# jameschapman19/cca_zoo

Measured on AMD Instinct MI355X. Metric: CCA fit()/sec at n=1e6 d=4096 k=64, higher is better.
Workload: dtype f32

## Files before the change

cca_zoo_amd/csrc/gram.hip:

```cpp
#include <algorithm>
#include <cstdio>
#include <cstdlib>
#include <cstring>
#include <thread>
#include <vector>

#include "hip_common.h"
#include "gram_map.h"

namespace ccz {

typedef float v16f32 __attribute__((ext_vector_type(16)));
typedef float v4f32 __attribute__((ext_vector_type(4)));
typedef double v4f64 __attribute__((ext_vector_type(4)));
typedef double v2f64 __attribute__((ext_vector_type(2)));

constexpr int BK = 16;

typedef const float __attribute__((address_space(1)))* gptr_f32;
typedef const double __attribute__((address_space(1)))* gptr_f64;

typedef unsigned int v4u32 __attribute__((ext_vector_type(4)));

constexpr int T32 = 256;
// ... 687 lines not shown
                                                      double* __restrict__ zero_me, int64_t nzero) {
  __shared__ int last;
  if (zero_me && blockIdx.y == 0)
    for (int64_t e = int64_t(blockIdx.x) * 256 + threadIdx.x; e < nzero; e += int64_t(gridDim.x) * 256) zero_me[e] = 0.0;
  const int64_t j = int64_t(blockIdx.x) * 256 + threadIdx.x;
  const int64_t r0 = int64_t(blockIdx.y) * rows_per_block;
  const int64_t r1 = min(n, r0 + rows_per_block);
  if (j < D) {
    int a = 0;
    while (a + 1 < cv.m && j >= cv.off[a + 1]) ++a;
    const float* X = cv.data[a] + (j - cv.off[a]);
    const int64_t ld = cv.ld[a];
    double a0 = 0.0, a1 = 0.0, a2 = 0.0, a3 = 0.0;
    int64_t r = r0;
    for (; r + 3 < r1; r += 4) {
      a0 += double(X[(r + 0) * ld]); a1 += double(X[(r + 1) * ld]);
      a2 += double(X[(r + 2) * ld]); a3 += double(X[(r + 3) * ld]);
    }
    for (; r < r1; ++r) a0 += double(X[r * ld]);
    st_shared(part + int64_t(blockIdx.y) * D + j, (a0 + a1) + (a2 + a3));
  }
  asm volatile("s_waitcnt vmcnt(0)" ::: "memory");
  __syncthreads();
  if (threadIdx.x == 0)
    last = __hip_atomic_fetch_add(counters + blockIdx.x, 1u, __ATOMIC_RELAXED, __HIP_MEMORY_SCOPE_AGENT) == gridDim.y - 1 ? 1 : 0;
  __syncthreads();
  if (!last) return;
  if (threadIdx.x == 0) __hip_atomic_store(counters + blockIdx.x, 0u, __ATOMIC_RELAXED, __HIP_MEMORY_SCOPE_AGENT);
  if (j >= D) return;
  double t0 = 0.0, t1 = 0.0, t2 = 0.0, t3 = 0.0;
  int rb = 0;
  const int nrb = int(gridDim.y);
  for (; rb + 3 < nrb; rb += 4) {
    t0 += ld_shared(part + int64_t(rb) * D + j); t1 += ld_shared(part + int64_t(rb + 1) * D + j);
    t2 += ld_shared(part + int64_t(rb + 2) * D + j); t3 += ld_shared(part + int64_t(rb + 3) * D + j);
  }
  for (; rb < nrb; ++rb) t0 += ld_shared(part + int64_t(rb) * D + j);
  const double sj = (t0 + t1) + (t2 + t3);
  sums[j] = sj;
  pilot[j] = float(sj / double(n));
}

__global__ void k_pilot_from_sums(const double* __restrict__ s, int64_t D, double inv_n, float* __restrict__ pilot) {
  const int64_t j = int64_t(blockIdx.x) * blockDim.x + threadIdx.x;
  if (j < D) pilot[j] = float(s[j] * inv_n);
}

__global__ void k_pilot_fixup(double* __restrict__ G, int64_t D, const double* __restrict__ s_launch, double n,
                              const float* __restrict__ pilot) {
  const int64_t i = blockIdx.y;
  const int64_t j = i + int64_t(blockIdx.x) * blockDim.x + threadIdx.x;
  if (j >= D) return;
  const double pi = double(pilot[i]), pj = double(pilot[j]);
  G[i * D + j] += pi * s_launch[j] + pj * s_launch[i] - n * pi * pj;
}

__global__ __launch_bounds__(256) void k_gram_reduce(const float* __restrict__ partial, const GramTile* __restrict__ tiles, int ntiles,
                                                     int64_t ksplit, double* __restrict__ G, int64_t ldg) {
  const int tile = blockIdx.y;
  const GramTile t = tiles[tile];
  const int e = blockIdx.x * 256 + threadIdx.x;
  const int i = e >> 8, j = e & 255;
  if (i >= t.wa || j >= t.wb) return;
  double acc = 0.0;
  const float* p = partial + int64_t(tile) * (T32 * T32) + e;
  for (int64_t c = 0; c < ksplit; ++c) acc += double(p[c * int64_t(ntiles) * (T32 * T32)]);
  G[(t.out_row + i) * ldg + t.out_col + j] += acc;
}

__global__ void k_vec_add(double* __restrict__ dst, const double* __restrict__ src, int64_t n) {
  const int64_t j = int64_t(blockIdx.x) * blockDim.x + threadIdx.x;
  if (j < n) dst[j] += src[j];
}

namespace {

struct Panel {
  int view;
  int64_t col0, width, gcol0;
};

struct TileTable {
  GramTile* dev = nullptr;
  int ntiles = 0;
  bool fast = true;
  std::vector<unsigned char> diag;
};

template <typename T>
TileTable build_tile_table(ccz_ctx* c, const ccz_view* views, int n_views, void** tile_cache) {
  Impl* im = impl(c);
  hipStream_t st = stream(c);
  constexpr bool is32 = sizeof(T) == 4;
  const int tile = is32 ? T32 : T64;
  std::vector<Panel> panels;
  int64_t g0 = 0;
  bool fast = true;
  for (int v = 0; v < n_views; ++v) {
    for (int64_t c0 = 0; c0 < views[v].cols; c0 += tile)
      panels.push_back({v, c0, std::min<int64_t>(tile, views[v].cols - c0), g0 + c0});
    if (views[v].cols % tile != 0) fast = false;
    if ((views[v].ld * sizeof(T)) % 16 != 0) fast = false;
    if (reinterpret_cast<uintptr_t>(views[v].data) % 16 != 0) fast = false;
    g0 += views[v].cols;
  }
  std::vector<GramTile> tiles;
  const int np = int(panels.size());
// ... 121 lines not shown
template <typename T>
RowPlan plan_rows(ccz_ctx* c, const ccz_view* views, int n_views, int64_t n, int ntiles, bool fast) {
  Impl* im = impl(c);
  constexpr bool is32 = sizeof(T) == 4;
  static const int map_mode = [] { const char* e = getenv("CCZ_GRAM_MAP"); return e ? atoi(e) : 1; }();
  const int ncu = std::max(1, im->props.multiProcessorCount);
  static const int64_t rows_env = [] { const char* e = getenv("CCZ_GRAM_ROWS"); return e ? atoll(e) : 0LL; }();
  int64_t max_rows = rows_env > 0 ? rows_env : 16384;
  if (fast) {
    int64_t cap = max_rows;
    for (int v = 0; v < n_views; ++v)
      cap = std::min<int64_t>(cap, ((int64_t(1) << 31) - 1) / (views[v].ld * int64_t(sizeof(T))) - 128);
    if (cap < 256) fast = false; else max_rows = cap;
  }
  const int64_t gran = (is32 && fast) ? FB * FR : BK;
  int64_t rows_per_wg;
  {
    const int64_t kmin = std::max<int64_t>(1, (n + max_rows - 1) / max_rows);
    const int64_t kmax = std::max<int64_t>(kmin, std::min<int64_t>(n / 256, 8192));
    double best = 1e300;
    int64_t best_k = kmin;
    for (int64_t ks = kmin; ks <= kmax; ++ks) {
      const int64_t rows = ((n + ks - 1) / ks + gran - 1) / gran * gran;
      const bool big = int64_t(ntiles) * ks >= 16 * int64_t(ncu);
      int64_t rounds;
      double penalty = 1.0;
      if (big && map_mode == 1 && ks % 8 == 0) rounds = ((ks / 8) * int64_t(ntiles) + ncu / 8 - 1) / (ncu / 8);
      else if (big) { rounds = (int64_t((ntiles + 7) / 8) * ks + ncu / 8 - 1) / (ncu / 8); if (map_mode == 1) penalty = 1.03; }
      else rounds = (int64_t(ntiles) * ks + ncu - 1) / ncu;
      const double cost = penalty * double(rounds) * double(rows + 320);
      if (cost < best) { best = cost; best_k = ks; }
    }
    rows_per_wg = ((n + best_k - 1) / best_k + gran - 1) / gran * gran;
  }
  const int64_t ksplit = (n + rows_per_wg - 1) / rows_per_wg;
  const bool sliced = int64_t(ntiles) * ksplit >= 16 * int64_t(ncu);
  const bool xchunks = sliced && map_mode == 1 && ksplit % 8 == 0;
  const int per_xcd = xchunks ? -1 : (sliced ? (ntiles + 7) / 8 : 0);
  const int64_t nblocks = xchunks ? int64_t(ntiles) * ksplit : (sliced ? int64_t(8) * per_xcd * ksplit : int64_t(ntiles) * ksplit);
  if (nblocks > 0x7fffffffLL) fail(CCZ_EUNSUP, "gram: grid too large");

  RowPlan rp;
  rp.rows_per_wg = rows_per_wg;
  rp.ksplit = ksplit;
  rp.nblocks = nblocks;
  rp.per_xcd = per_xcd;
  rp.sliced = sliced;
  rp.fast = fast;
  return rp;
}

template <typename T>
bool launch_moments(ccz_ctx* c, const ccz_view* views, int n_views, int64_t n, double* G, double* s, int64_t D,
                    bool time_it, void** tile_cache = nullptr, int pilot_mode = 0) {
  Impl* im = impl(c);
  hipStream_t st = stream(c);
  constexpr bool is32 = sizeof(T) == 4;
  const int tile = is32 ? T32 : T64;
  const TileTable tt = build_tile_table<T>(c, views, n_views, tile_cache);
  GramTile* d_tiles = tt.dev;
  const int ntiles = tt.ntiles;
  const RowPlan rp = plan_rows<T>(c, views, n_views, n, ntiles, tt.fast);
  const bool fast = rp.fast;
  const int64_t rows_per_wg = rp.rows_per_wg, ksplit = rp.ksplit, nblocks = rp.nblocks;
  const int per_xcd = rp.per_xcd;
  const bool sliced = rp.sliced;
  const int ncu = std::max(1, im->props.multiProcessorCount);
  const size_t lds_bytes = size_t(2) * 2 * BK * tile * sizeof(T);
  static const int pilot_env = [] { const char* e = getenv("CCZ_GRAM_PILOT"); return e ? atoi(e) : -1; }();
  if (pilot_env == 0 || pilot_env == 1) pilot_mode = pilot_env == 1 ? 2 : 0;
  if (!is32) pilot_mode = 0;
  bool split = false;
  if (is32) {
    static const int route_env = [] {
      const char* e = getenv("CCZ_K1_ROUTE");
      if (!e) return 0;
      if (!strcmp(e, "fp32")) return int(CCZ_K1_FP32);
      if (!strcmp(e, "bf16x2")) return int(CCZ_K1_BF16X2);
      return 0;
    }();
    const int route = c->k1_route != CCZ_K1_AUTO ? c->k1_route : route_env;
    split = (route == CCZ_K1_BF16X2 || (route == CCZ_K1_AUTO && gram_split_worthwhile(n, D))) && n_views <= 16;
    if (split) pilot_mode = 2;
  }
  c->last_route = !is32 ? CCZ_K1_FP64 : (split ? CCZ_K1_BF16X2 : CCZ_K1_FP32);
  static const double pilot_thr = [] { const char* e = getenv("CCZ_GRAM_PILOT_RATIO"); return e ? atof(e) : 2.0; }();
  double* s_launch = s;
  double* sq = nullptr;
  if (pilot_mode != 0) {
    s_launch = static_cast<double*>(dev_alloc(c, size_t(D) * 8 * (pilot_mode == 1 ? 2 : 1)));
    zero(c, s_launch, size_t(D) * 8 * (pilot_mode == 1 ? 2 : 1));
    if (pilot_mode == 1) sq = s_launch + D;
  }
  if (time_it) CCZ_HIP(hipEventRecord(im->ev[2], st));
  int64_t off = 0;
  float* pilot = nullptr;
  if (split) {
    const int64_t nsamp = std::min<int64_t>(n, 2048), stride = n / nsamp;
    double* samp = static_cast<double*>(dev_alloc(c, size_t(D) * 8));
    zero(c, samp, size_t(D) * 8);
    for (int v = 0; v < n_views; ++v) {
      const int64_t colblocks = (views[v].cols + 255) / 256;
      int64_t rpb = 256;
      while (rpb > 16 && colblocks * ((nsamp + rpb - 1) / rpb) < 2 * int64_t(ncu)) rpb /= 2;
      dim3 grid((unsigned)colblocks, (unsigned)((nsamp + rpb - 1) / rpb));
      hipLaunchKernelGGL((k_colsum<T, false>), grid, dim3(256), 0, st, static_cast<const T*>(views[v].data), nsamp, views[v].cols,
                         views[v].ld * stride, samp + off, static_cast<double*>(nullptr), rpb);
      off += views[v].cols;
    }
    pilot = static_cast<float*>(dev_alloc(c, size_t(D) * 4));
    hipLaunchKernelGGL(k_pilot_from_sums, dim3((unsigned)((D + 255) / 256)), dim3(256), 0, st, samp, D, 1.0 / double(nsamp), pilot);
    dev_free(c, samp);
  }
  for (int v = 0; v < n_views && !split; ++v) {
    const int64_t colblocks = (views[v].cols + 255) / 256;
    int64_t rpb = 2048;
    while (rpb > 64 && colblocks * ((n + rpb - 1) / rpb) < 4 * int64_t(ncu)) rpb /= 2;
    dim3 grid((unsigned)colblocks, (unsigned)((n + rpb - 1) / rpb));
    if (sq)
      hipLaunchKernelGGL((k_colsum<T, true>), grid, dim3(256), 0, st, static_cast<const T*>(views[v].data), n, views[v].cols,
                         views[v].ld, s_launch + off, sq + off, rpb);
    else
      hipLaunchKernelGGL((k_colsum<T, false>), grid, dim3(256), 0, st, static_cast<const T*>(views[v].data), n, views[v].cols,
                         views[v].ld, s_launch + off, static_cast<double*>(nullptr), rpb);
    off += views[v].cols;
  }
  CCZ_LAUNCH_CHECK();
  if (time_it) CCZ_HIP(hipEventRecord(im->ev[3], st));
  bool use_pilot = pilot_mode == 2;
  if (pilot_mode == 1) {
    std::vector<double> hs(size_t(2) * D);
    d2h(c, hs.data(), s_launch, size_t(2) * D * 8);
    double worst = 0.0;
    for (int64_t j = 0; j < D; ++j) {
      const double mu = hs[j] / double(n), var = hs[D + j] / double(n) - mu * mu;
      if (!std::isfinite(mu) || !std::isfinite(var)) continue;
      const double sd = var > 0.0 ? std::sqrt(var) : 0.0;
      const double ratio = std::fabs(mu) <= pilot_thr * sd ? 0.0 : (sd > 0.0 ? std::fabs(mu) / sd : 1e300);
      if (ratio > worst) worst = ratio;
    }
    use_pilot = worst > pilot_thr;
  }
  if (use_pilot && !split) {
    pilot = static_cast<float*>(dev_alloc(c, size_t(D) * 4));
    hipLaunchKernelGGL(k_pilot_from_sums, dim3((unsigned)((D + 255) / 256)), dim3(256), 0, st, s_launch, D, 1.0 / double(n), pilot);
  }

  if (time_it) CCZ_HIP(hipEventRecord(im->ev[0], st));
  static const int impl_sel = [] { const char* e = getenv("CCZ_GRAM_IMPL"); return e ? atoi(e) : 1; }();
  static const int fifo_pilot_env = [] { const char* e = getenv("CCZ_GRAM_FIFO_PILOT"); return e ? atoi(e) : 1; }();
  const int64_t n_main = n / (FB * FR) * (FB * FR);
  const bool fifo_pilot = is32 && fast && impl_sel != 0 && use_pilot && fifo_pilot_env != 0 && sliced && n_main >= rows_per_wg;
  float* partial = nullptr;
  const bool staged32 = is32 && !(fast && impl_sel != 0 && !use_pilot) && !fifo_pilot;
  if (staged32 && ksplit >= 2 && !sliced && !split) {
    static const int64_t partial_cap = [] { const char* e = getenv("CCZ_GRAM_PARTIAL_MB"); return (e ? atoll(e) : 192LL) << 20; }();
    const int64_t bytes = ksplit * int64_t(ntiles) * T32 * T32 * 4;
    if (bytes <= partial_cap) partial = static_cast<float*>(dev_alloc(c, size_t(bytes)));
  }
  if (split) {
    gram_split_f32(c, views, n_views, n, G, D, pilot, s_launch, time_it);
  } else if (is32) {
    if (fifo_pilot) {
      const size_t fifo_bytes = size_t(4) * FR * FSLOT;
      CCZ_HIP(hipFuncSetAttribute(reinterpret_cast<const void*>(&k_gram_f32_fifo<true>), hipFuncAttributeMaxDynamicSharedMemorySize, int(fifo_bytes)));
      hipLaunchKernelGGL(k_gram_f32_fifo<true>, dim3((unsigned)nblocks), dim3(256), fifo_bytes, st, d_tiles, ntiles, per_xcd, ksplit, n_main,
                         rows_per_wg, G, D, pilot);
      if (n_main < n) {
        CCZ_HIP(hipFuncSetAttribute(reinterpret_cast<const void*>(&k_gram_f32<true>), hipFuncAttributeMaxDynamicSharedMemorySize, int(lds_bytes)));
        hipLaunchKernelGGL(k_gram_f32<true>, dim3((unsigned)ntiles), dim3(256), lds_bytes, st, d_tiles, ntiles, 0, int64_t(1), n, int64_t(FB * FR), G, D,
                           pilot, static_cast<float*>(nullptr), n_main);
      }
    } else if (fast && impl_sel != 0 && !use_pilot) {
      const size_t fifo_bytes = size_t(4) * FR * FSLOT;
      CCZ_HIP(hipFuncSetAttribute(reinterpret_cast<const void*>(&k_gram_f32_fifo<false>), hipFuncAttributeMaxDynamicSharedMemorySize, int(fifo_bytes)));
      hipLaunchKernelGGL(k_gram_f32_fifo<false>, dim3((unsigned)nblocks), dim3(256), fifo_bytes, st, d_tiles, ntiles, per_xcd, ksplit, n, rows_per_wg, G, D,
                         static_cast<const float*>(nullptr));
    } else if (fast) {
      CCZ_HIP(hipFuncSetAttribute(reinterpret_cast<const void*>(&k_gram_f32<true>), hipFuncAttributeMaxDynamicSharedMemorySize, int(lds_bytes)));
      hipLaunchKernelGGL(k_gram_f32<true>, dim3((unsigned)nblocks), dim3(256), lds_bytes, st, d_tiles, ntiles, per_xcd, ksplit, n, rows_per_wg, G, D, pilot, partial, int64_t(0));
    } else {
      CCZ_HIP(hipFuncSetAttribute(reinterpret_cast<const void*>(&k_gram_f32<false>), hipFuncAttributeMaxDynamicSharedMemorySize, int(lds_bytes)));
      hipLaunchKernelGGL(k_gram_f32<false>, dim3((unsigned)nblocks), dim3(256), lds_bytes, st, d_tiles, ntiles, per_xcd, ksplit, n, rows_per_wg, G, D, pilot, partial, int64_t(0));
    }
  } else {
    static const int impl64 = [] { const char* e = getenv("CCZ_GRAM64_IMPL"); return e ? atoi(e) : 1; }();
    if (fast && impl64 != 0) {
      const size_t fifo_bytes = size_t(4) * FR * FSLOT;
      CCZ_HIP(hipFuncSetAttribute(reinterpret_cast<const void*>(&k_gram_f64_fifo), hipFuncAttributeMaxDynamicSharedMemorySize, int(fifo_bytes)));
      hipLaunchKernelGGL(k_gram_f64_fifo, dim3((unsigned)nblocks), dim3(256), fifo_bytes, st, d_tiles, ntiles, per_xcd, ksplit, n, rows_per_wg, G, D);
    } else if (fast) {
      CCZ_HIP(hipFuncSetAttribute(reinterpret_cast<const void*>(&k_gram_f64<true>), hipFuncAttributeMaxDynamicSharedMemorySize, int(lds_bytes)));
      hipLaunchKernelGGL(k_gram_f64<true>, dim3((unsigned)nblocks), dim3(256), lds_bytes, st, d_tiles, ntiles, per_xcd, ksplit, n, rows_per_wg, G, D);
    } else {
      CCZ_HIP(hipFuncSetAttribute(reinterpret_cast<const void*>(&k_gram_f64<false>), hipFuncAttributeMaxDynamicSharedMemorySize, int(lds_bytes)));
      hipLaunchKernelGGL(k_gram_f64<false>, dim3((unsigned)nblocks), dim3(256), lds_bytes, st, d_tiles, ntiles, per_xcd, ksplit, n, rows_per_wg, G, D);
    }
  }
  CCZ_LAUNCH_CHECK();
  if (partial) {
    hipLaunchKernelGGL(k_gram_reduce, dim3(256, (unsigned)ntiles), dim3(256), 0, st, partial, d_tiles, ntiles, ksplit, G, D);
    CCZ_LAUNCH_CHECK();
    dev_free(c, partial);
  }
  if (time_it) CCZ_HIP(hipEventRecord(im->ev[1], st));
  if (use_pilot) {
    if (D > 65535) fail(CCZ_EUNSUP, "gram: pilot fix-up supports D <= 65535");
    hipLaunchKernelGGL(k_pilot_fixup, dim3((unsigned)((D + 255) / 256), (unsigned)D), dim3(256), 0, st, G, D, s_launch, double(n), pilot);
  }
  if (s_launch != s) hipLaunchKernelGGL(k_vec_add, dim3((unsigned)((D + 255) / 256)), dim3(256), 0, st, s, s_launch, D);
  CCZ_LAUNCH_CHECK();
  if (time_it) {
    CCZ_HIP(hipEventSynchronize(im->ev[1]));
    float g = 0.f, cs = 0.f;
    CCZ_HIP(hipEventElapsedTime(&g, im->ev[0], im->ev[1]));
    CCZ_HIP(hipEventElapsedTime(&cs, im->ev[2], im->ev[3]));
    c->last_gram_ms += g;
    c->last_colsum_ms += cs;
  }
  c->last_pilot = use_pilot ? 1 : 0;
  if (pilot) dev_free(c, pilot);
  if (s_launch != s) dev_free(c, s_launch);
  return use_pilot;
}

bool ensure_pipe(ccz_ctx* c, size_t bytes) {
  Impl* im = impl(c);
  if (!im->copy_stream) {
    if (hipStreamCreateWithFlags(&im->copy_stream, hipStreamNonBlocking) != hipSuccess) { (void)hipGetLastError(); im->copy_stream = nullptr; return false; }
    for (int i = 0; i < 4; ++i)
      if (hipEventCreateWithFlags(&im->pipe_ev[i], hipEventDisableTiming) != hipSuccess) { (void)hipGetLastError(); return false; }
  }
  for (int i = 0; i < 4; ++i) if (!im->pipe_ev[i]) return false;
  if (im->pin_cap >= bytes) return true;
  for (int i = 0; i < 2; ++i) {
    if (im->pin_buf[i]) (void)hipHostFree(im->pin_buf[i]);
    im->pin_buf[i] = nullptr;
  }
  im->pin_cap = 0;
  for (int i = 0; i < 2; ++i)
    if (hipHostMalloc(&im->pin_buf[i], bytes, hipHostMallocDefault) != hipSuccess) {
      (void)hipGetLastError();
      for (int j = 0; j < 2; ++j) { if (im->pin_buf[j]) (void)hipHostFree(im->pin_buf[j]); im->pin_buf[j] = nullptr; }
      return false;
    }
  im->pin_cap = bytes;
  return true;
}

void pack_rows(char* dst, const ccz_view* views, int n_views, size_t es, int64_t r0, int64_t rows, int nthreads) {
  auto work = [&](int64_t a, int64_t b) {
    size_t off = 0;
    for (int v = 0; v < n_views; ++v) {
      const size_t rb = size_t(views[v].cols) * es, ldb = size_t(views[v].ld) * es;
      const char* src = static_cast<const char*>(views[v].data) + size_t(r0 + a) * ldb;
      char* d = dst + off + size_t(a) * rb;
      if (rb == ldb) memcpy(d, src, size_t(b - a) * rb);
      else for (int64_t r = a; r < b; ++r, src += ldb, d += rb) memcpy(d, src, rb);
      off += size_t(rows) * rb;
// ... 116 lines not shown
  out->partial = static_cast<float*>(dev_alloc(c, size_t(bytes)));
  out->tile_plan = fifo_plan_ok ? fifo_plan_dev : nullptr;
  if (!colsum_pilot_f32(c, views, n_views, n, D, out->colsum, out->pilot, nullptr, 0)) {
    gram_partials_release(c, out);
    return false;
  }
  const size_t lds_bytes = size_t(2) * 2 * BK * T32 * sizeof(float);
  if (fifo_plan_ok) {
    const size_t fifo_bytes = size_t(4) * FR * FSLOT;
    CCZ_HIP(hipFuncSetAttribute(reinterpret_cast<const void*>(&k_gram_f32_fifo_small<true>), hipFuncAttributeMaxDynamicSharedMemorySize, int(fifo_bytes)));
    hipLaunchKernelGGL(k_gram_f32_fifo_small<true>, dim3((unsigned)fifo_wgs), dim3(256), fifo_bytes, st, tt.dev, tt.ntiles, out->tile_plan, n,
                       out->partial, out->pilot);
  } else if (rp.fast) {
    CCZ_HIP(hipFuncSetAttribute(reinterpret_cast<const void*>(&k_gram_f32<true>), hipFuncAttributeMaxDynamicSharedMemorySize, int(lds_bytes)));
    hipLaunchKernelGGL(k_gram_f32<true>, dim3((unsigned)rp.nblocks), dim3(256), lds_bytes, st, tt.dev, tt.ntiles, rp.per_xcd, rp.ksplit, n, rp.rows_per_wg,
                       static_cast<double*>(nullptr), D, out->pilot, out->partial, int64_t(0));
  } else {
    CCZ_HIP(hipFuncSetAttribute(reinterpret_cast<const void*>(&k_gram_f32<false>), hipFuncAttributeMaxDynamicSharedMemorySize, int(lds_bytes)));
    hipLaunchKernelGGL(k_gram_f32<false>, dim3((unsigned)rp.nblocks), dim3(256), lds_bytes, st, tt.dev, tt.ntiles, rp.per_xcd, rp.ksplit, n, rp.rows_per_wg,
                       static_cast<double*>(nullptr), D, out->pilot, out->partial, int64_t(0));
  }
  CCZ_LAUNCH_CHECK();
  out->tiles = tt.dev;
  out->ntiles = tt.ntiles;
  out->ksplit = rp.ksplit;
  c->last_pilot = 1;
  c->last_route = CCZ_K1_FP32;
  return true;
}

void gram_partials_release(ccz_ctx* c, GramPartials* gp) {
  if (gp->planes) dev_free(c, gp->planes);
  if (gp->msq) dev_free(c, const_cast<double*>(gp->msq));
  gp->planes = nullptr; gp->msq = nullptr;
  if (gp->partial) dev_free(c, gp->partial);
  if (gp->pilot) dev_free(c, gp->pilot);
  if (gp->colsum) dev_free(c, gp->colsum);
  gp->partial = nullptr; gp->pilot = nullptr; gp->colsum = nullptr; gp->tile_plan = nullptr;
}

void moments_impl(ccz_ctx* c, int dtype, const ccz_view* views, int n_views, int64_t n_rows, bool on_device,
                  double* moments, bool accumulate, int pilot_mode, bool time_it) {
  if (!views || n_views < 1 || !moments) fail(CCZ_EINVAL, "moments: null argument");
  if (dtype != CCZ_F32 && dtype != CCZ_F64) fail(CCZ_EUNSUP, "moments: dtype must be CCZ_F32 or CCZ_F64");
  if (n_rows < 0) fail(CCZ_EINVAL, "moments: negative row count");
  int64_t D = 0;
  for (int v = 0; v < n_views; ++v) {
    if (views[v].cols < 1 || views[v].ld < views[v].cols || (!views[v].data && n_rows > 0))
      fail(CCZ_EINVAL, "moments: view %d is malformed (cols=%lld ld=%lld)", v, (long long)views[v].cols, (long long)views[v].ld);
    D += views[v].cols;
  }
  double* G = moments;
  double* s = moments + D * D;
  if (!accumulate) zero(c, moments, size_t(D * D + D) * 8);
  c->last_gram_ms = 0.0;
  c->last_colsum_ms = 0.0;
  if (n_rows == 0) return;
  const size_t es = dtype == CCZ_F32 ? 4 : 8;
  if (on_device) {
    if (dtype == CCZ_F32) launch_moments<float>(c, views, n_views, n_rows, G, s, D, time_it, nullptr, pilot_mode);
    else launch_moments<double>(c, views, n_views, n_rows, G, s, D, time_it, nullptr, 0);
    return;
  }
  int64_t row_bytes = 0;
  for (int v = 0; v < n_views; ++v) row_bytes += views[v].cols * int64_t(es);
  const int64_t chunk_mb = [] { const char* e = getenv("CCZ_H2D_CHUNK_MB"); return e ? std::max<int64_t>(1, atoll(e)) : 1024LL; }();
  const int n_threads = [] {
    const char* e = getenv("CCZ_H2D_THREADS");
    if (e) return std::max(1, atoi(e));
    return int(std::max(1u, std::min(8u, std::thread::hardware_concurrency())));
  }();
  int64_t chunk = std::max<int64_t>(64, (chunk_mb << 20) / row_bytes / 64 * 64);
  chunk = std::min(chunk, n_rows);
  const bool piped = n_rows * row_bytes >= (int64_t(64) << 20) && n_rows > chunk / 2 && ensure_pipe(c, size_t(chunk) * row_bytes);
  const int nslots = piped ? 2 : 1;
  Impl* im = impl(c);
  bool src_pinned = piped;
  for (int v = 0; v < n_views && src_pinned; ++v) {
    hipPointerAttribute_t at{};
    if (hipPointerGetAttributes(&at, views[v].data) != hipSuccess) { (void)hipGetLastError(); src_pinned = false; break; }
    src_pinned = at.type == hipMemoryTypeHost;
    if (src_pinned) {
      const char* last = static_cast<const char*>(views[v].data) + (size_t(n_rows - 1) * views[v].ld + views[v].cols) * es - 1;
      hipPointerAttribute_t a2{};
      if (hipPointerGetAttributes(&a2, last) != hipSuccess) { (void)hipGetLastError(); src_pinned = false; }
      else src_pinned = a2.type == hipMemoryTypeHost;
    }
  }
  static const bool pinned_direct = [] { const char* e = getenv("CCZ_H2D_PINNED_DIRECT"); return !e || atoi(e) != 0; }();
  src_pinned = src_pinned && pinned_direct;
  std::vector<void*> stage(size_t(nslots) * n_views, nullptr);
  std::vector<ccz_view> dv(size_t(nslots) * n_views);
  void* tile_tab[2] = {nullptr, nullptr};
  auto cleanup = [&] {
    (void)hipStreamSynchronize(stream(c));
    if (piped) (void)hipStreamSynchronize(im->copy_stream);
    for (void* p : stage) if (p) dev_free(c, p);
    for (void* p : tile_tab) if (p) dev_free(c, p);
  };
  try {
    for (int sl = 0; sl < nslots; ++sl)
      for (int v = 0; v < n_views; ++v) {
        stage[sl * n_views + v] = dev_alloc(c, size_t(chunk) * views[v].cols * es);
        dv[sl * n_views + v] = ccz_view{stage[sl * n_views + v], views[v].cols, views[v].cols};
      }
    if (piped) {
      CCZ_HIP(hipEventRecord(im->pipe_ev[2], stream(c)));
      CCZ_HIP(hipStreamWaitEvent(im->copy_stream, im->pipe_ev[2], 0));
    }
    int64_t ci = 0;
    const int chunk_mode = pilot_mode == 1 ? 2 : pilot_mode;
    const int64_t min_chunk = std::max<int64_t>(64, ((int64_t(128) << 20) / row_bytes) / 64 * 64);
    int64_t rows = 0;
// ... 48 lines not shown
```

cca_zoo_amd/csrc/gram_split.hip:

```cpp
#include <algorithm>
#include <cstdio>
#include <cstdlib>
#include <cstring>
#include <vector>

#include "hip_common.h"
#include "gram_map.h"
#include "split_mma.h"

namespace ccz {

constexpr int SP_MAXV = 16;

struct SplitPanel {
  int32_t view;
  int32_t col0;
  int32_t width;
  int32_t gcol0;
};

struct SplitViews {
  const float* data[SP_MAXV];
  int64_t ld[SP_MAXV];
};
// ... 128 lines not shown
  extern __shared__ __attribute__((aligned(16))) char smem[];
  const WorkItem wi = locate_work(blockIdx.x, ntiles, per_xcd, ksplit);
  if (!wi.valid) return;
  const SplitTile t = tiles[wi.tile];
  const int64_t s0 = wi.chunk * steps_per_wg;
  const int64_t s1 = min(ksteps, s0 + steps_per_wg);
  if (s0 >= s1) return;
  const int tid = threadIdx.x, lane = tid & 63;
  const int wave = __builtin_amdgcn_readfirstlane(tid >> 6);
  const int wr = wave >> 1, wc = wave & 1;

  sp_v16f32 acc[4][4];
#pragma unroll
  for (int i = 0; i < 4; ++i)
#pragma unroll
    for (int j = 0; j < 4; ++j)
#pragma unroll
      for (int r = 0; r < 16; ++r) acc[i][j][r] = 0.f;
  const char* srcA = planes + (int64_t(t.pa) * ksteps + s0) * SP_PSTEP;
  const char* srcB = planes + (int64_t(t.pb) * ksteps + s0) * SP_PSTEP;
  const int nsteps = int(s1 - s0);
  int qr = wr, qc = wc, ti0 = 0, ti1 = 4;
  bool sym = false;
  if (t.diag && wr == wc) {
    sym = true;
    split_mma_core<1>(acc, smem, srcA, srcB, nsteps, wave, lane, qr, qc);
  } else if (t.diag && wr == 0) {
    ti1 = 2;
    split_mma_core<2>(acc, smem, srcA, srcB, nsteps, wave, lane, qr, qc);
  } else if (t.diag) {
    qr = 0; qc = 1; ti0 = 2;
    split_mma_core<3>(acc, smem, srcA, srcB, nsteps, wave, lane, qr, qc);
  } else {
    split_mma_core<0>(acc, smem, srcA, srcB, nsteps, wave, lane, qr, qc);
  }

  float* pt = partial + (wi.chunk * int64_t(ntiles) + wi.tile) * int64_t(SP_T * SP_T);
#pragma unroll
  for (int ti = 0; ti < 4; ++ti) {
    if (ti < ti0 || ti >= ti1) continue;
    float* prow = pt + (qr * 128 + ti * 32 + (lane & 31)) * SP_T + qc * 128 + 4 * (lane >> 5);
#pragma unroll
    for (int tj = 0; tj < 4; ++tj) {
      if (sym && tj < ti) continue;
#pragma unroll
      for (int g = 0; g < 4; ++g) {
        const sp_v4f32 v = {acc[ti][tj][4 * g], acc[ti][tj][4 * g + 1], acc[ti][tj][4 * g + 2], acc[ti][tj][4 * g + 3]};
        *reinterpret_cast<sp_v4f32*>(prow + tj * 32 + 8 * g) = v;
      }
    }
  }
}

__global__ __launch_bounds__(256) void k_split_reduce(const float* __restrict__ partial, const SplitTile* __restrict__ tiles, int ntiles,
                                                      int64_t ksplit, double* __restrict__ G, int64_t ldg, const double* __restrict__ msq) {
  const int tile = blockIdx.y;
  const SplitTile t = tiles[tile];
  const int e = (blockIdx.x * 256 + threadIdx.x) * 4;
  const int i = e >> 8, j = e & 255;
  if (i >= t.wa || j >= t.wb) return;
  double a0 = 0.0, a1 = 0.0, a2 = 0.0, a3 = 0.0;
  const float* p = partial + int64_t(tile) * (SP_T * SP_T) + e;
  const int64_t stride = int64_t(ntiles) * (SP_T * SP_T);
  for (int64_t c = 0; c < ksplit; ++c) {
    const sp_v4f32 v = __builtin_nontemporal_load(reinterpret_cast<const sp_v4f32*>(p + c * stride));
    a0 += double(v[0]); a1 += double(v[1]); a2 += double(v[2]); a3 += double(v[3]);
  }
  const double a[4] = {a0, a1, a2, a3};
  double* g = G + (int64_t(t.out_row) + i) * ldg + t.out_col + j;
#pragma unroll
  for (int q = 0; q < 4; ++q) {
    if (j + q >= t.wb) break;
    if (t.diag && j + q < i) continue;
    double v = a[q];
    if (t.diag && i == j + q) v += msq[t.out_row + i];
    g[q] += v;
  }
}

namespace {

std::vector<std::pair<int, int>> split_tile_order(int np) {
  std::vector<std::pair<int, int>> full, dg, rest;
  for (int I = 0; I < np; I += 4)
    for (int J = (I / 8) * 8; J < np; J += 8) {
      std::vector<std::pair<int, int>> blk;
      bool has_diag = false;
      for (int i = I; i < std::min(np, I + 4); ++i)
        for (int j = std::max(i, J); j < std::min(np, J + 8); ++j) { blk.emplace_back(i, j); has_diag = has_diag || i == j; }
      for (const auto& ij : blk) {
        if (blk.size() == 32 && !has_diag) full.push_back(ij);
        else (ij.first == ij.second ? dg : rest).push_back(ij);
      }
    }
  full.insert(full.end(), dg.begin(), dg.end());
  full.insert(full.end(), rest.begin(), rest.end());
  return full;
}

}

size_t split_scratch_budget(ccz_ctx* c) {
  const char* e = getenv("CCZ_SPLIT_SCRATCH_GB");
  const double env_gb = e ? atof(e) : 48.0;
  const double cap = 0.4 * double(impl(c)->props.totalGlobalMem);
  return size_t(std::max(8.0 * 1048576.0, std::min(env_gb * 1073741824.0, cap)));
}

static int split_rows_per_block(int64_t rows_pad, int64_t npanels, int ncu) {
  int rb = SP_RB;
  while (rb > 32 && ((rows_pad + rb - 1) / rb) * npanels < 2 * int64_t(ncu)) rb /= 2;
  return rb;
}

struct SplitTables {
  const SplitPanel* panels;
  const SplitTile* tiles;
  const GramTile* gtiles;
  int np, ntiles;
};

static SplitTables split_tables(ccz_ctx* c, const int64_t* cols, int n_views) {
  Impl* im = impl(c);
  uint64_t key = 1469598103934665603ull;
  auto mix = [&](uint64_t v) { key ^= v; key *= 1099511628211ull; };
  mix(uint64_t(n_views));
  int np = 0;
  for (int v = 0; v < n_views; ++v) { mix(uint64_t(cols[v])); np += int((cols[v] + SP_T - 1) / SP_T); }
  SplitTables tb;
// ... 170 lines not shown
      char* end = nullptr;
      const double f = strtod(q, &end);
      if (end == q) break;
      if (f > 0.0 && f < 1.0) fr.push_back(f);
      q = *end == ',' ? end + 1 : end;
      if (end && *end != ',' ) break;
    }
  }
  std::vector<int64_t> out;
  const int64_t T = (rows + unit - 1) / unit;
  int64_t used = 0;
  if (T >= 8 && fr.size() <= 6) {
    for (double f : fr) {
      const int64_t u = std::max<int64_t>(1, int64_t(f * double(T) + 0.5));
      if (used + u >= T) break;
      out.push_back(u * unit);
      used += u;
    }
  }
  out.push_back(rows - used * unit);
  return out;
}

static hipStream_t split_side_stream(ccz_ctx* c) {
  Impl* im = impl(c);
  const int ncu = std::max(1, im->props.multiProcessorCount);
  const char* e = getenv("CCZ_SPLIT_PIPE_CUS");
  const int cus = e ? atoi(e) : 64;
  if (im->split_stream_tried && cus == im->split_stream_req) return im->split_stream;
  if (im->split_stream) {
    (void)hipStreamSynchronize(im->split_stream);
    (void)hipStreamDestroy(im->split_stream);
    im->split_stream = nullptr;
  }
  im->split_stream_tried = true;
  im->split_stream_req = cus;
  im->split_stream_cus = 0;
  hipStream_t st = nullptr;
  if (cus > 0 && cus < ncu && ncu % 8 == 0) {
    const int stride = std::max(1, ncu / cus);
    std::vector<uint32_t> mask(size_t((ncu + 31) / 32), 0u);
    int set = 0;
    for (int i = 0; i < ncu; ++i)
      if ((i / 8) % stride == 0) { mask[size_t(i >> 5)] |= 1u << (i & 31); ++set; }
    if (hipExtStreamCreateWithCUMask(&st, uint32_t(mask.size()), mask.data()) == hipSuccess) im->split_stream_cus = set;
    else { (void)hipGetLastError(); st = nullptr; }
  }
  if (!st && hipStreamCreateWithFlags(&st, hipStreamNonBlocking) != hipSuccess) { (void)hipGetLastError(); st = nullptr; }
  im->split_stream = st;
  return st;
}

void gram_split_f32(ccz_ctx* c, const ccz_view* views, int n_views, int64_t n, double* G, int64_t D, const float* pilot, double* colsum,
                    bool time_it) {
  Impl* im = impl(c);
  hipStream_t st = stream(c);
  if (n_views > SP_MAXV) fail(CCZ_EUNSUP, "gram (split route): more than %d views", SP_MAXV);
  if (D > 0x7fffffffLL - 256) fail(CCZ_EUNSUP, "gram (split route): stacked width too large");
  int64_t cols[SP_MAXV];
  for (int v = 0; v < n_views; ++v) cols[v] = views[v].cols;
  const SplitTables tb = split_tables(c, cols, n_views);
  SplitViews vws{};
  const bool aligned = split_views_arg(views, n_views, &vws);
  const int np = tb.np, ntiles = tb.ntiles;
  const SplitTile* d_tiles = tb.tiles;
  double* msq = static_cast<double*>(dev_alloc(c, size_t(D) * 8));
  char* planes = nullptr;
  float* partial = nullptr;
  bool side_busy = false;
  auto release = [&] {
    if (side_busy && im->split_stream) (void)hipStreamSynchronize(im->split_stream);
    if (partial) dev_free(c, partial);
    if (planes) dev_free(c, planes);
    dev_free(c, msq);
  };
  try {
    const int ncu = std::max(1, im->props.multiProcessorCount);
    const char* rows_env = getenv("CCZ_SPLIT_ROWS");
    const int64_t max_steps = std::max<int64_t>(1, (rows_env ? atoll(rows_env) : 16384LL) / SP_K);
    const double per_row = double(np) * SP_PSTEP / SP_K + double(ntiles) * (SP_T * SP_T * 4) / double(max_steps * SP_K);
    const size_t budget = split_scratch_budget(c);
    int64_t launch_rows = int64_t(double(budget) / per_row) / (max_steps * SP_K) * (max_steps * SP_K);
    launch_rows = std::max<int64_t>(launch_rows, max_steps * SP_K);
    const int64_t n_launch = (n + launch_rows - 1) / launch_rows;
    launch_rows = ((n + n_launch - 1) / n_launch + SP_K - 1) / SP_K * SP_K;
    const size_t fifo_bytes = size_t(SP_NST) * SP_STAGE;
    sp_allow_lds(reinterpret_cast<const void*>(&k_gram_bf16x2), c->device, int(fifo_bytes));
    c->last_split_ms = c->last_mfma_ms = c->last_reduce_ms = 0.0;
    size_t planes_cap = 0, partial_cap = 0;
    bool launched = false;
   retry_smaller:
    try {
    for (int64_t r0 = 0; r0 < n; r0 += launch_rows) {
      const int64_t rows = std::min(launch_rows, n - r0);
      std::vector<int64_t> piece_rows = split_pieces(rows, max_steps * SP_K);
      hipStream_t side = piece_rows.size() > 1 ? split_side_stream(c) : nullptr;
      if (!side) piece_rows.assign(1, rows);
      const int npc = int(piece_rows.size());
      struct Piece { int64_t r0, rows, ksteps, slice0; size_t planes_off; SplitRowPlan rp; };
      std::vector<Piece> pcs;
      pcs.resize(size_t(npc));
      size_t planes_bytes = 0;
      int64_t slices = 0;
      {
        int64_t off = 0;
        for (int p = 0; p < npc; ++p) {
          Piece& pc = pcs[size_t(p)];
          pc.r0 = r0 + off;
          pc.rows = piece_rows[size_t(p)];
          pc.ksteps = (pc.rows + SP_K - 1) / SP_K;
          pc.rp = split_row_plan(pc.ksteps, ntiles, max_steps, ncu);
          pc.planes_off = planes_bytes;
          pc.slice0 = slices;
          planes_bytes += size_t(np) * size_t(pc.ksteps) * SP_PSTEP;
          slices += pc.rp.ksplit;
          off += pc.rows;
        }
      }
      const size_t partial_bytes = size_t(slices) * size_t(ntiles) * (SP_T * SP_T * 4);
      if (planes_bytes > planes_cap) { if (planes) dev_free(c, planes); planes = static_cast<char*>(dev_alloc(c, planes_bytes)); planes_cap = planes_bytes; }
      if (partial_bytes > partial_cap) { if (partial) dev_free(c, partial); partial = static_cast<float*>(dev_alloc(c, partial_bytes)); partial_cap = partial_bytes; }
      const size_t nev = size_t(4 * npc);
      while (im->sp_ev.size() < nev) {
        hipEvent_t e = nullptr;
        CCZ_HIP(hipEventCreate(&e));
        im->sp_ev.push_back(e);
      }
      hipEvent_t* ev = im->sp_ev.data();
      launched = true;
      side_busy = side != nullptr;
      zero(c, msq, size_t(D) * 8);
      if (time_it) CCZ_HIP(hipEventRecord(ev[0], st));
      launch_split_pass(c, tb, vws, aligned, pcs[0].r0, pcs[0].rows, pcs[0].ksteps, pilot, planes, msq, colsum, st);
      if (time_it || side) CCZ_HIP(hipEventRecord(ev[1], st));
      if (side) {
        CCZ_HIP(hipStreamWaitEvent(side, ev[1], 0));
        for (int p = 1; p < npc; ++p) {
          const Piece& pc = pcs[size_t(p)];
          if (time_it) CCZ_HIP(hipEventRecord(ev[4 * p - 1], side));
          launch_split_pass(c, tb, vws, aligned, pc.r0, pc.rows, pc.ksteps, pilot, planes + pc.planes_off, msq, colsum, side);
          CCZ_HIP(hipEventRecord(ev[4 * p], side));
        }
      }
      for (int p = 0; p < npc; ++p) {
        const Piece& pc = pcs[size_t(p)];
        if (p > 0) {
          CCZ_HIP(hipStreamWaitEvent(st, ev[4 * p], 0));
          if (time_it) CCZ_HIP(hipEventRecord(ev[4 * p + 1], st));
        }
        hipLaunchKernelGGL(k_gram_bf16x2, dim3((unsigned)pc.rp.nblocks), dim3(256), fifo_bytes, st, d_tiles, ntiles, pc.rp.per_xcd, pc.rp.ksplit,
                           planes + pc.planes_off, pc.ksteps, pc.rp.steps_per_wg, partial + pc.slice0 * int64_t(ntiles) * (SP_T * SP_T));
        if (time_it) CCZ_HIP(hipEventRecord(ev[4 * p + 2], st));
      }
      side_busy = false;
      hipLaunchKernelGGL(k_split_reduce, dim3(64, (unsigned)ntiles), dim3(256), 0, st, partial, d_tiles, ntiles, slices, G, D, msq);
      CCZ_LAUNCH_CHECK();
      if (time_it) {
        hipEvent_t last = ev[4 * npc - 1];
        CCZ_HIP(hipEventRecord(last, st));
        CCZ_HIP(hipEventSynchronize(last));
        float a = 0.f;
        CCZ_HIP(hipEventElapsedTime(&a, ev[0], ev[1]));
        c->last_split_ms += a;
        CCZ_HIP(hipEventElapsedTime(&a, ev[1], ev[2]));
        c->last_mfma_ms += a;
        for (int p = 1; p < npc; ++p) {
          CCZ_HIP(hipEventElapsedTime(&a, ev[4 * p - 1], ev[4 * p]));
          c->last_split_ms += a;
          CCZ_HIP(hipEventElapsedTime(&a, ev[4 * p + 1], ev[4 * p + 2]));
          c->last_mfma_ms += a;
        }
        CCZ_HIP(hipEventElapsedTime(&a, ev[4 * (npc - 1) + 2], last));
        c->last_reduce_ms += a;
      }
    }
    } catch (const Error& e) {
      if (e.code != CCZ_ENOMEM || launched || launch_rows <= max_steps * SP_K) throw;
      if (planes) { dev_free(c, planes); planes = nullptr; }
      if (partial) { dev_free(c, partial); partial = nullptr; }
      planes_cap = partial_cap = 0;
      launch_rows = std::max<int64_t>(max_steps * SP_K, launch_rows / 2 / (max_steps * SP_K) * (max_steps * SP_K));
      goto retry_smaller;
    }
  } catch (...) {
    release();
    throw;
  }
  release();
}

}
```

cca_zoo_amd/csrc/hip_common.h:

```cpp
#pragma once

#include <hip/hip_runtime.h>

#include <utility>
#include <vector>

#include "ops.h"

namespace ccz {

struct PoolBlock {
  void* p;
  size_t bytes;
  bool used;
};

struct GraphEntry {
  uint64_t key;
  hipGraphExec_t exec;
  uint64_t tick;
};

struct Impl {
  hipDeviceProp_t props;
// ... 16 lines not shown
  hipEvent_t small_ev[kSmallSlots] = {};
  int small_next = 0;
  hipStream_t aux_stream = nullptr;
  hipEvent_t aux_ev[2] = {nullptr, nullptr};
  hipEvent_t bj_ev[8] = {};
  struct TileTab { uint64_t hash; size_t bytes; void* dev; uint64_t tick; };
  std::vector<TileTab> tile_tabs;
  int* loss_status = nullptr;
  int* loss_status_dev = nullptr;
  hipEvent_t xs_ev[2] = {nullptr, nullptr};
  hipEvent_t wait_ev = nullptr;
  void* d2h_pin = nullptr;
  void* d2h_pin_dev = nullptr;
  hipEvent_t d2h_tev[2] = {nullptr, nullptr};
  static constexpr size_t kD2hPinBytes = size_t(4) << 20;
  void* deferred_event = nullptr;
  hipEvent_t defer_own_ev = nullptr;
  bool adopted = false;
  std::vector<std::pair<void*, void*>> chain_sync;
  int chain_cap = 0;
  void* chain_dbg = nullptr;
  struct K1Plan { uint64_t key; void* dev; int wgs; };
  std::vector<K1Plan> k1_plans;
  std::vector<hipEvent_t> sp_ev;
  hipStream_t split_stream = nullptr;
  bool split_stream_tried = false;
  int split_stream_req = 0;
  int split_stream_cus = 0;
  struct SplitTab { uint64_t key; void* panels; void* tiles; void* gtiles; int np, ntiles; };
  std::vector<SplitTab> split_tabs;
  std::vector<std::pair<void*, void*>> colsum_sync;
  void* xchg_buf = nullptr;
  size_t xchg_cap = 0;
  hipStream_t xchg_stream = nullptr;
  hipEvent_t xchg_ev[3] = {nullptr, nullptr, nullptr};
  void* comm = nullptr;
  int comm_world = 0, comm_rank = -1;
};

inline Impl* impl(ccz_ctx* c) { return static_cast<Impl*>(c->impl); }
inline hipStream_t stream(ccz_ctx* c) { return static_cast<hipStream_t>(c->stream); }

#define CCZ_HIP(expr)                                                                         \
  do {                                                                                        \
    hipError_t _e = (expr);                                                                   \
    if (_e != hipSuccess)                                                                     \
      ::ccz::fail(CCZ_EHIP, "%s failed: %s (%s:%d)", #expr, hipGetErrorString(_e), __FILE__, \
                  __LINE__);                                                                  \
  } while (0)

#define CCZ_LAUNCH_CHECK() CCZ_HIP(hipGetLastError())

#ifdef __HIPCC__
typedef unsigned long long __attribute__((address_space(1)))* gu64_ptr;
typedef unsigned __attribute__((address_space(1)))* gu32_ptr;
__device__ __forceinline__ double ld_shared(const double* p) {
  const unsigned long long u = __hip_atomic_load((gu64_ptr)(reinterpret_cast<uintptr_t>(p)), __ATOMIC_RELAXED, __HIP_MEMORY_SCOPE_AGENT);
  return __longlong_as_double((long long)u);
}
__device__ __forceinline__ void st_shared(double* p, double v) {
  __hip_atomic_store((gu64_ptr)(reinterpret_cast<uintptr_t>(p)), (unsigned long long)__double_as_longlong(v), __ATOMIC_RELAXED,
                     __HIP_MEMORY_SCOPE_AGENT);
}
typedef unsigned int ccz_v4u32 __attribute__((ext_vector_type(4)));
__device__ __forceinline__ void st_shared2(double* p, double a, double b) {
  ccz_v4u32 v;
  v[0] = unsigned(__double2loint(a)); v[1] = unsigned(__double2hiint(a));
  v[2] = unsigned(__double2loint(b)); v[3] = unsigned(__double2hiint(b));
  asm volatile("global_store_dwordx4 %0, %1, off sc1\n\ts_nop 1" : : "v"(p), "v"(v) : "memory");
}
#endif

uint64_t graph_key_mix(uint64_t h, uint64_t v);
void graph_run_fn(ccz_ctx* c, uint64_t key, const std::function<void()>& fn);
void sync_short(ccz_ctx* c);

int jacobi_rows_block(ccz_ctx* c, int64_t p, int64_t q, double* W, int64_t ldw, double* Q, int64_t qc, int64_t ldq, int max_sweeps);

void moments_blocks(ccz_ctx* c, bool pack, double* mom, int64_t D, const int64_t* dims, int m, double* packed, int which,
                    void* on_stream);

struct GramTile {
  const void* a;
  const void* b;
  int64_t lda, ldb;
  int64_t out_row, out_col;
  int32_t wa, wb;
  int32_t diag;
  int32_t pad_;
};

struct GramPartials {
  const GramTile* tiles = nullptr;
  int ntiles = 0;
  int64_t ksplit = 0;
  float* partial = nullptr;
  float* pilot = nullptr;
  double* colsum = nullptr;
  int* tile_plan = nullptr;
  const double* msq = nullptr;
  char* planes = nullptr;
};
bool gram_split_worthwhile(int64_t n, int64_t D);
void gram_split_f32(ccz_ctx* c, const ccz_view* views, int n_views, int64_t n, double* G, int64_t D, const float* pilot, double* colsum,
                    bool time_it);
bool gemm_split_pair_eligible(int64_t M, int64_t N, int64_t K, int64_t K1, int64_t nsplit, const void* A1, int64_t lda1, const void* A2,
                              int64_t lda2, const void* C1, int64_t ldc1, const void* C2, int64_t ldc2);
void gemm_split_pair(ccz_ctx* c, int64_t M, int64_t N, int64_t K, int64_t K1, float alpha, const float* alpha_dev, const float* A1, int64_t lda1,
                     const float* A2, int64_t lda2, const float* gamma32, const double* corr, const double* mean, float* C1,
                     int64_t ldc1, float* C2, int64_t ldc2, int64_t nsplit);
bool project_split_eligible(ccz_ctx* c, int64_t n, int64_t d, int64_t k, int64_t ld, const void* X, int64_t ldo);
void project_split(ccz_ctx* c, const float* X, int64_t n, int64_t d, int64_t ld, const double* mean, const double* W, int64_t k, float* out,
                   int64_t ldo);
bool gram_partials_f32(ccz_ctx* c, const ccz_view* views, int n_views, int64_t n, GramPartials* out);
bool colsum_pilot_f32(ccz_ctx* c, const ccz_view* views, int n_views, int64_t n, int64_t D, double* colsum, float* pilot, double* zero_me,
                      int64_t nzero);
bool gram_partials_split_f32(ccz_ctx* c, const ccz_view* views, int n_views, int64_t n, GramPartials* out);
void gram_partials_release(ccz_ctx* c, GramPartials* gp);

void moments_impl(ccz_ctx* c, int dtype, const ccz_view* views, int n_views, int64_t n_rows,
                  bool on_device, double* moments, bool accumulate, int pilot_mode = 1, bool time_it = true);
void h2d_small(ccz_ctx* c, void* dst, const void* src, size_t bytes);
void gemm_mixed(ccz_ctx* c, int dtype, int64_t M, int64_t N, int64_t K, double alpha, const void* A,
                int64_t lda, const double* B, int64_t ldb, double beta, void* C, int64_t ldc,
                const double* bias_row );

bool gemm_f32_big_eligible(int64_t M, int64_t N, int64_t K, int64_t lda, int64_t ldb, int64_t ldc, const void* A,
                           const void* C);
void gemm_f32_big(ccz_ctx* c, int64_t M, int64_t N, int64_t K, double alpha, const float* A, int64_t lda,
                  const double* B, int64_t ldb, double beta, float* C, int64_t ldc, const double* bias_row);

bool gemm_f32_fifo_split_eligible(int64_t M, int64_t N, int64_t K, int64_t nsplit, const void* C1, int64_t ldc1, const void* C2,
                                  int64_t ldc2);
void gemm_f32_fifo_split(ccz_ctx* c, int64_t M, int64_t N, int64_t K, float alpha, const float* A, int64_t lda, const float* B32,
                         const float* bias32, float* C1, int64_t ldc1, float* C2, int64_t ldc2, int64_t nsplit);

bool gemm_f32_fifo_pair_eligible(int64_t M, int64_t N, int64_t K, int64_t K1, int64_t nsplit, const void* A1, int64_t lda1, const void* A2,
                                 int64_t lda2, const void* C1, int64_t ldc1, const void* C2, int64_t ldc2);
void gemm_f32_fifo_pair(ccz_ctx* c, int64_t M, int64_t N, int64_t K, int64_t K1, float alpha, const float* alpha_dev, const float* A1,
                        int64_t lda1, const float* A2, int64_t lda2, const float* B32, const double* bias64, float* C1, int64_t ldc1,
                        float* C2, int64_t ldc2, int64_t nsplit);

bool gemm_f64_big_eligible(bool tA, bool tB, int64_t M, int64_t N, int64_t K, const double* A, int64_t lda,
                           const double* B, int64_t ldb, const double* C, int64_t ldc);
void gemm_f64_big(ccz_ctx* c, bool tA, bool tB, int64_t M, int64_t N, int64_t K, double alpha, const double* A,
                  int64_t lda, const double* B, int64_t ldb, double beta, double* C, int64_t ldc, bool lower_only);

bool gemm_f64_skinny_eligible(bool tA, bool tB, int64_t M, int64_t N, int64_t K, const double* A, int64_t lda,
                              const double* B, int64_t ldb);
void gemm_f64_skinny(ccz_ctx* c, bool tA, int64_t M, int64_t N, int64_t K, double alpha, const double* A, int64_t lda,
                     const double* B, int64_t ldb, double beta, double* C, int64_t ldc);

void cholinv_batched(ccz_ctx* c, int count, double* const* A, const int64_t* lda, const int64_t* d, double* const* L,
                     const int64_t* ldl, double* const* X, const int64_t* ldx, double* const* T, int* info_dev);
void trinv_batched(ccz_ctx* c, int count, const double* const* L, const int64_t* ldl, const int64_t* d, double* const* X,
                   const int64_t* ldx, const double* const* T);
void copy_lower(ccz_ctx* c, int64_t d, const double* src, int64_t lds_, double* dst, int64_t ldd);
struct MultiGemmArgs {
// ... 16 lines not shown
```

Measured before the change: 5.522.

## Fuse pilot fix-up and G zeroing into split-route reduce kernel

On the split (bf16x2) route, the separate pilot fix-up pass over G is folded into the final reduce kernel. For a fresh single-chunk fit, the reduce stores G directly and zeroes the untouched lower and transposed regions itself, instead of requiring a full D×D memset first. This drops two full passes over the D×D fp64 Gram matrix (the memset and the fix-up read-modify-write). In exchange the reduce kernel gets more complex and adds extra stores in off-diagonal transpose regions.

```diff
diff --git a/cca_zoo_amd/csrc/gram.hip b/cca_zoo_amd/csrc/gram.hip
--- a/cca_zoo_amd/csrc/gram.hip
+++ b/cca_zoo_amd/csrc/gram.hip
@@ -763,7 +763,7 @@
   const int64_t j = i + int64_t(blockIdx.x) * blockDim.x + threadIdx.x;
   if (j >= D) return;
   const double pi = double(pilot[i]), pj = double(pilot[j]);
-  G[i * D + j] += pi * s_launch[j] + pj * s_launch[i] - n * pi * pj;
+  G[i * D + j] += pilot_fix(pi, pj, s_launch[i], s_launch[j], n);
 }
 
 __global__ __launch_bounds__(256) void k_gram_reduce(const float* __restrict__ partial, const GramTile* __restrict__ tiles, int ntiles,
@@ -991,7 +991,7 @@
 
 template <typename T>
 bool launch_moments(ccz_ctx* c, const ccz_view* views, int n_views, int64_t n, double* G, double* s, int64_t D,
-                    bool time_it, void** tile_cache = nullptr, int pilot_mode = 0) {
+                    bool time_it, void** tile_cache = nullptr, int pilot_mode = 0, bool fresh = false) {
   Impl* im = impl(c);
   hipStream_t st = stream(c);
   constexpr bool is32 = sizeof(T) == 4;
@@ -1023,6 +1023,7 @@
     if (split) pilot_mode = 2;
   }
   c->last_route = !is32 ? CCZ_K1_FP64 : (split ? CCZ_K1_BF16X2 : CCZ_K1_FP32);
+  if (fresh && !split) zero(c, G, size_t(D) * size_t(D) * 8);
   static const double pilot_thr = [] { const char* e = getenv("CCZ_GRAM_PILOT_RATIO"); return e ? atof(e) : 2.0; }();
   double* s_launch = s;
   double* sq = nullptr;
@@ -1098,7 +1099,7 @@
     if (bytes <= partial_cap) partial = static_cast<float*>(dev_alloc(c, size_t(bytes)));
   }
   if (split) {
-    gram_split_f32(c, views, n_views, n, G, D, pilot, s_launch, time_it);
+    gram_split_f32(c, views, n_views, n, G, D, pilot, s_launch, time_it, fresh);
   } else if (is32) {
     if (fifo_pilot) {
       const size_t fifo_bytes = size_t(4) * FR * FSLOT;
@@ -1143,7 +1144,7 @@
     dev_free(c, partial);
   }
   if (time_it) CCZ_HIP(hipEventRecord(im->ev[1], st));
-  if (use_pilot) {
+  if (use_pilot && !split) {
     if (D > 65535) fail(CCZ_EUNSUP, "gram: pilot fix-up supports D <= 65535");
     hipLaunchKernelGGL(k_pilot_fixup, dim3((unsigned)((D + 255) / 256), (unsigned)D), dim3(256), 0, st, G, D, s_launch, double(n), pilot);
   }
@@ -1366,13 +1367,17 @@
   }
   double* G = moments;
   double* s = moments + D * D;
-  if (!accumulate) zero(c, moments, size_t(D * D + D) * 8);
+  const bool fresh = !accumulate && on_device && dtype == CCZ_F32 && n_rows > 0;
+  if (!accumulate) {
+    if (fresh) zero(c, s, size_t(D) * 8);
+    else zero(c, moments, size_t(D * D + D) * 8);
+  }
   c->last_gram_ms = 0.0;
   c->last_colsum_ms = 0.0;
   if (n_rows == 0) return;
   const size_t es = dtype == CCZ_F32 ? 4 : 8;
   if (on_device) {
-    if (dtype == CCZ_F32) launch_moments<float>(c, views, n_views, n_rows, G, s, D, time_it, nullptr, pilot_mode);
+    if (dtype == CCZ_F32) launch_moments<float>(c, views, n_views, n_rows, G, s, D, time_it, nullptr, pilot_mode, fresh);
     else launch_moments<double>(c, views, n_views, n_rows, G, s, D, time_it, nullptr, 0);
     return;
   }
diff --git a/cca_zoo_amd/csrc/gram_split.hip b/cca_zoo_amd/csrc/gram_split.hip
--- a/cca_zoo_amd/csrc/gram_split.hip
+++ b/cca_zoo_amd/csrc/gram_split.hip
@@ -204,12 +204,20 @@
   }
 }
 
+template <bool STORE>
 __global__ __launch_bounds__(256) void k_split_reduce(const float* __restrict__ partial, const SplitTile* __restrict__ tiles, int ntiles,
-                                                      int64_t ksplit, double* __restrict__ G, int64_t ldg, const double* __restrict__ msq) {
+                                                      int64_t ksplit, double* __restrict__ G, int64_t ldg, const double* __restrict__ msq,
+                                                      const float* __restrict__ pilot, const double* __restrict__ colsum, double n_fix) {
   const int tile = blockIdx.y;
   const SplitTile t = tiles[tile];
   const int e = (blockIdx.x * 256 + threadIdx.x) * 4;
   const int i = e >> 8, j = e & 255;
+  if (STORE && !t.diag && i < t.wb) {
+    double* z = G + (int64_t(t.out_col) + i) * ldg + t.out_row + j;
+#pragma unroll
+    for (int q = 0; q < 4; ++q)
+      if (j + q < t.wa) z[q] = 0.0;
+  }
   if (i >= t.wa || j >= t.wb) return;
   double a0 = 0.0, a1 = 0.0, a2 = 0.0, a3 = 0.0;
   const float* p = partial + int64_t(tile) * (SP_T * SP_T) + e;
@@ -220,13 +228,24 @@
   }
   const double a[4] = {a0, a1, a2, a3};
   double* g = G + (int64_t(t.out_row) + i) * ldg + t.out_col + j;
+  const int gi = t.out_row + i;
+  double pi = 0.0, si = 0.0;
+  if (pilot) { pi = double(pilot[gi]); si = colsum[gi]; }
 #pragma unroll
   for (int q = 0; q < 4; ++q) {
     if (j + q >= t.wb) break;
-    if (t.diag && j + q < i) continue;
+    if (t.diag && j + q < i) {
+      if (STORE) g[q] = 0.0;
+      continue;
+    }
     double v = a[q];
-    if (t.diag && i == j + q) v += msq[t.out_row + i];
-    g[q] += v;
+    if (t.diag && i == j + q) v += msq[gi];
+    if (!STORE) v = g[q] + v;
+    if (pilot) {
+      const int gj = t.out_col + j + q;
+      v += pilot_fix(pi, double(pilot[gj]), si, colsum[gj], n_fix);
+    }
+    g[q] = v;
   }
 }
 
@@ -503,9 +522,10 @@
 }
 
 void gram_split_f32(ccz_ctx* c, const ccz_view* views, int n_views, int64_t n, double* G, int64_t D, const float* pilot, double* colsum,
-                    bool time_it) {
+                    bool time_it, bool fresh) {
   Impl* im = impl(c);
   hipStream_t st = stream(c);
+  if (pilot && !colsum) fail(CCZ_EINVAL, "gram (split route): a pilot shift needs the column sums to undo it");
   if (n_views > SP_MAXV) fail(CCZ_EUNSUP, "gram (split route): more than %d views", SP_MAXV);
   if (D > 0x7fffffffLL - 256) fail(CCZ_EUNSUP, "gram (split route): stacked width too large");
   int64_t cols[SP_MAXV];
@@ -604,7 +624,16 @@
         if (time_it) CCZ_HIP(hipEventRecord(ev[4 * p + 2], st));
       }
       side_busy = false;
-      hipLaunchKernelGGL(k_split_reduce, dim3(64, (unsigned)ntiles), dim3(256), 0, st, partial, d_tiles, ntiles, slices, G, D, msq);
+      const bool last = r0 + rows >= n;
+      const float* fix_pilot = last ? pilot : nullptr;
+      if (fresh && r0 == 0 && last) {
+        hipLaunchKernelGGL(k_split_reduce<true>, dim3(64, (unsigned)ntiles), dim3(256), 0, st, partial, d_tiles, ntiles, slices, G, D, msq,
+                           fix_pilot, colsum, double(n));
+      } else {
+        if (fresh && r0 == 0) zero(c, G, size_t(D) * size_t(D) * 8);
+        hipLaunchKernelGGL(k_split_reduce<false>, dim3(64, (unsigned)ntiles), dim3(256), 0, st, partial, d_tiles, ntiles, slices, G, D, msq,
+                           fix_pilot, colsum, double(n));
+      }
       CCZ_LAUNCH_CHECK();
       if (time_it) {
         hipEvent_t last = ev[4 * npc - 1];
diff --git a/cca_zoo_amd/csrc/hip_common.h b/cca_zoo_amd/csrc/hip_common.h
--- a/cca_zoo_amd/csrc/hip_common.h
+++ b/cca_zoo_amd/csrc/hip_common.h
@@ -92,6 +92,9 @@
 #define CCZ_LAUNCH_CHECK() CCZ_HIP(hipGetLastError())
 
 #ifdef __HIPCC__
+__device__ __forceinline__ double pilot_fix(double pi, double pj, double si, double sj, double n) {
+  return __builtin_fma(-(n * pi), pj, __builtin_fma(sj, pi, si * pj));
+}
 typedef unsigned long long __attribute__((address_space(1)))* gu64_ptr;
 typedef unsigned __attribute__((address_space(1)))* gu32_ptr;
 __device__ __forceinline__ double ld_shared(const double* p) {
@@ -143,7 +146,7 @@
 };
 bool gram_split_worthwhile(int64_t n, int64_t D);
 void gram_split_f32(ccz_ctx* c, const ccz_view* views, int n_views, int64_t n, double* G, int64_t D, const float* pilot, double* colsum,
-                    bool time_it);
+                    bool time_it, bool fresh);
 bool gemm_split_pair_eligible(int64_t M, int64_t N, int64_t K, int64_t K1, int64_t nsplit, const void* A1, int64_t lda1, const void* A2,
                               int64_t lda2, const void* C1, int64_t ldc1, const void* C2, int64_t ldc2);
 void gemm_split_pair(ccz_ctx* c, int64_t M, int64_t N, int64_t K, int64_t K1, float alpha, const float* alpha_dev, const float* A1, int64_t lda1,
```

Result: no change. 5.535 (median of 6 runs) (+0.2%).
